# bibymaths/phoskintime

Measured on AMD Instinct MI355X. Metric: ODE-solve replicas/sec (32-state distributive, 14 tp), higher is better.
Workload: dtype f64

## Files before the change

### phoskintime_amd/csrc/pk_dist_fast.hpp

```cpp
#pragma once
#include "pk_dist_rows.hpp"
#include "pk_env.hpp"

namespace pk {

template <int G, int RPL>
__device__ __forceinline__ double site_sum(const double (&s)[RPL], int lane) { return gsum<G>(tree_sum(s), lane); }

enum { PK_DM_NONE = 0, PK_DM_SUM = 1, PK_DM_FULL = 2 };
__host__ __device__ __forceinline__ int dist_metric_class(const SolveArgs& A) {
  return !A.metric ? PK_DM_NONE : (A.metric_id == PK_METRIC_TOTAL_SIGNAL || A.metric_id == PK_METRIC_MEAN_ACTIVITY) ? PK_DM_SUM : PK_DM_FULL;
}
template <bool CLIP, bool NORM, bool FLAT, bool SOL, int MC>
struct DistFixed {
  static constexpr int SLOT_MC = MC;
  static constexpr bool LITERAL = false;
  __host__ __device__ static __forceinline__ bool clip(const SolveArgs&) { return CLIP; }
  __host__ __device__ static __forceinline__ bool normalize(const SolveArgs&) { return NORM; }
  __host__ __device__ static __forceinline__ bool flat(const SolveArgs&) { return FLAT; }
  __host__ __device__ static __forceinline__ bool sol(const SolveArgs&) { return SOL; }
  __host__ __device__ static __forceinline__ int mclass(const SolveArgs&) { return MC; }
  static bool matches(const SolveArgs& A) {
    return (A.clip != 0) == CLIP && (A.normalize != 0) == NORM && (A.flat != nullptr) == FLAT && (A.sol != nullptr) == SOL && dist_metric_class(A) == MC;
  }
};
struct DistAny {
  static constexpr int SLOT_MC = PK_DM_FULL;
  static constexpr bool LITERAL = true;
  __host__ __device__ static __forceinline__ bool clip(const SolveArgs& A) { return A.clip != 0; }
  __host__ __device__ static __forceinline__ bool normalize(const SolveArgs& A) { return A.normalize != 0; }
  __host__ __device__ static __forceinline__ bool flat(const SolveArgs& A) { return A.flat != nullptr; }
  __host__ __device__ static __forceinline__ bool sol(const SolveArgs& A) { return A.sol != nullptr; }
  __host__ __device__ static __forceinline__ int mclass(const SolveArgs& A) { return dist_metric_class(A); }
  static bool matches(const SolveArgs&) { return true; }
};
using DistSolSum = DistFixed<true, false, false, true, PK_DM_SUM>;
using DistSolOnly = DistFixed<true, false, false, true, PK_DM_NONE>;
using DistFlatOnly = DistFixed<true, false, true, false, PK_DM_NONE>;

template <int RPL, int MC, bool RES = false> constexpr int dist_fast_slots() {
  return MC == PK_DM_FULL ? 3 * RPL + (RES ? 4 : 6) : MC == PK_DM_SUM ? 2 * RPL + 1 : 2 * RPL;
}

template <int RPL, bool PARK, int NT> struct Parked;
template <int RPL, int NT> struct Parked<RPL, false, NT> {
  double v[3 * RPL + 6];
  __device__ __forceinline__ explicit Parked(double*) {}
  template <int K> __device__ __forceinline__ double get() const { return v[K]; }
  template <int K> __device__ __forceinline__ void set(double x) { v[K] = x; }
  __device__ __forceinline__ void fence() {}
};
template <int RPL, int NT> struct Parked<RPL, true, NT> {
  typedef __attribute__((address_space(3))) double lds_double;
  lds_double* base;
  __device__ __forceinline__ explicit Parked(double* lds) : base((lds_double*)lds + threadIdx.x) {}
  template <int K> __device__ __forceinline__ double get() const { return base[K * NT]; }
  template <int K> __device__ __forceinline__ void set(double x) { base[K * NT] = x; }
  __device__ __forceinline__ void fence() { asm volatile("" : "+v"(base)); }
};
template <int RPL, bool PARK, int NT = 256, class CFG = DistAny, bool RES = false>
constexpr size_t dist_fast_lds_bytes() { return PARK ? (size_t)(dist_fast_slots<RPL, CFG::SLOT_MC, RES>() + RPL) * NT * sizeof(double) : 0; }

constexpr int PK_DSCHED_K2 = 5, PK_DSCHED_K1 = 9;
constexpr int PK_HWREG_HW_ID = 4 | (31 << 11), PK_HWREG_HW_ID_WAVE = 4 | (3 << 11), PK_HWREG_XCC_ID = 20 | (31 << 11);

template <bool PACE> struct DistPace {
  __device__ __forceinline__ void enter(const SolveArgs&) {}
  __device__ __forceinline__ void step(int) const {}
};
template <> struct DistPace<true> {
  bool paced = false;
  __device__ __forceinline__ void enter(const SolveArgs& A) {
    const int sched = A.sched;
    if (sched != PK_DSCHED_OFF) {
      bool leader = false;
      if ((int)gridDim.x > A.R1) {
        if (sched & PK_DSCHED_LEAD_SLOT) leader = (int)blockIdx.x < A.R1 && __builtin_amdgcn_s_getreg(PK_HWREG_HW_ID_WAVE) == 0;
        if (sched & PK_DSCHED_LEAD_BLOCK) leader = leader || (int)blockIdx.x < A.R1 / 3;
      }
      if (leader) __builtin_amdgcn_s_setprio(3);
      paced = !leader && (sched & PK_DSCHED_LEVEL) != 0;
    }
  }
  __device__ __forceinline__ void step(const int k) const {
    if (paced) {
      if (__builtin_amdgcn_ballot_w64(k < PK_DSCHED_K2) != 0) __builtin_amdgcn_s_setprio(2);
      else if (__builtin_amdgcn_ballot_w64(k < PK_DSCHED_K1) != 0) __builtin_amdgcn_s_setprio(1);
      else __builtin_amdgcn_s_setprio(0);
    }
  }
};

struct DistTraceRec {
  unsigned long long t_entry, t_exit;
  unsigned block, hw_id, xcc_id, iters;
};
struct DistTraceBuf { DistTraceRec* rec; long long capacity; };
template <int TRACE> struct DistTrace;

template <int TRACE> struct DistWaveTrace {
  int witer = 0;
  __device__ __forceinline__ void enter() {
    const unsigned long long t0 = __builtin_amdgcn_s_memrealtime();
    const DistTraceBuf tb = DistTrace<TRACE>::get();
    if (threadIdx.x == 0 && tb.rec && (long long)blockIdx.x < tb.capacity) {
      DistTraceRec* r = tb.rec + blockIdx.x;
      r->t_entry = t0; r->t_exit = 0; r->block = blockIdx.x; r->iters = 0;
      r->hw_id = __builtin_amdgcn_s_getreg(PK_HWREG_HW_ID); r->xcc_id = __builtin_amdgcn_s_getreg(PK_HWREG_XCC_ID);
    }
  }
  __device__ __forceinline__ void step() { ++witer; }
  __device__ __forceinline__ void exit() const {
    int it = witer;
    for (int o = 32; o > 0; o >>= 1) { const int v = __shfl_xor(it, o); it = v > it ? v : it; }
    const DistTraceBuf tb = DistTrace<TRACE>::get();
    if (threadIdx.x == 0 && tb.rec && (long long)blockIdx.x < tb.capacity) {
      DistTraceRec* r = tb.rec + blockIdx.x;
      r->iters = (unsigned)it; r->t_exit = __builtin_amdgcn_s_memrealtime();
    }
  }
};
template <> struct DistWaveTrace<0> {
  __device__ __forceinline__ void enter() {}
  __device__ __forceinline__ void step() {}
  __device__ __forceinline__ void exit() const {}
};

template <int G, int RPL, int METHOD, bool PARK = false, int MINB = (PARK ? 2 : 1), int NT = 256, class CFG = DistAny, bool RES = false, int TRACE = 0>
__global__ __launch_bounds__(NT, MINB) void dist_fast_kernel(const SolveArgs A) {
  using Tab = ResolventTab<METHOD>;
  using Vec = Stg<RPL, RES>;
  static_assert(!TRACE || NT == 64, "the trace holds one record per workgroup: one wave each");
  DistWaveTrace<TRACE> trace;
  trace.enter();
  DistPace<PARK && NT == 64 && METHOD == PK_METHOD_LRP12> pace;
  pace.enter(A);
  extern __shared__ __align__(16) double park_lds[];
  Parked<RPL, PARK, NT> pk(park_lds);
  static_assert(dist_fast_lds_bytes<RPL, PARK, 64, CFG, RES>() * 4 * MINB <= 160 * 1024, "parked slots exceed the CU's LDS at this occupancy");
  constexpr int MCS = CFG::SLOT_MC;
  constexpr int NSL = dist_fast_slots<RPL, MCS, RES>(), FB = 3 * RPL + (RES ? 0 : 2);
  constexpr int K_SR = 0, K_DG = RPL, K_PS = 2 * RPL, K_PR = 3 * RPL, K_PP = 3 * RPL + 1, K_M1 = (MCS == PK_DM_FULL ? FB : 2 * RPL),
                K_M2 = FB + 1, K_MD = FB + 2, K_SH = FB + 3, K_Y = NSL;
  constexpr int RPB = NT / G;
  const int lane = lane_id();
  const int l = threadIdx.x & (G - 1);
  const long long rep = (long long)blockIdx.x * RPB + (threadIdx.x / G);
  if (rep >= A.B) return;
  const int n = A.n_sites, S = A.S, T = A.T;
  const int mclass = CFG::mclass(A);
  const double* __restrict__ th = A.theta + rep * A.P;

  const double cA = th[0], cB = th[1], cC = th[2];
  const bool isR = RES && l == 0, isP = RES && l == 1;
  const double w0 = isR ? cC : 1.0, k3 = isR ? cA : 0.0;
  double lsum = 0.0;
  static_for<RPL>([&](auto jc) {
    constexpr int j = decltype(jc)::value;
    const int i = l + G * j - (RES ? 2 : 0);
    const bool ok = i >= 0 && i < n;
    const double sr = ok ? th[4 + i] : 0.0;
    double dg = ok ? 1.0 + th[4 + n + i] : 1.0;
    if constexpr (RES && j == 0) dg = isR ? cB : isP ? -cC : dg;
    pk.template set<K_SR + j>(sr);
    pk.template set<K_DG + j>(dg);
    lsum += sr;
  });
  const double Dsum = th[3] + gsum<G>(lsum, lane);
  auto sites_only = [&](const auto& s) {
    double v[RPL];
#pragma unroll
    for (int j = 0; j < RPL; ++j) v[j] = s[j];
    v[0] = (isR || isP) ? 0.0 : v[0];
    return gsum<G>(tree_sum(v), lane);
  };

  const double* y0p = A.y0 + (A.y0_batched ? rep * S : 0);
  Vec y;
  if constexpr (!RES) { y.R() = y0p[0]; y.P() = y0p[1]; }
#pragma unroll
  for (int j = 0; j < RPL; ++j) {
    const int i = l + G * j;
    if constexpr (RES) y.s[j] = (i < S) ? y0p[i] : 0.0;
    else y.s[j] = (i < n) ? y0p[2 + i] : 0.0;
  }
  if constexpr (PARK) static_for<RPL>([&](auto jc) { constexpr int j = decltype(jc)::value; pk.template set<K_Y + j>(y.s[j]); });

  static_for<NSL - 2 * RPL>([&](auto kc) { pk.template set<K_PS + decltype(kc)::value>(0.0); });
  const int T5 = T > 5 ? T - 5 : 0;
  double* srow = CFG::sol(A) ? A.sol + rep * T * S + (RES ? 0 : 2) + l : nullptr;
  auto emit = [&](const int k, const Vec& v, auto nf) {
    constexpr bool nan_fill = decltype(nf)::value;
    double* fl = CFG::flat(A) ? A.flat + rep * A.F : nullptr;
    bool clip_now = CFG::clip(A);
    if constexpr (!CFG::LITERAL && !nan_fill) if (clip_now) clip_now = __builtin_amdgcn_ballot_w64(sign_or(v) < 0) != 0;
    auto val = [&](double x, int state) {
      if (nan_fill) return __builtin_nan("");
      double r = (CFG::LITERAL && CFG::clip(A)) ? ((x < 0.0) ? 0.0 : x) : x;
      if (CFG::normalize(A)) r *= 1.0 / y0p[state];
      return r;
    };
    Vec c = v;
    if constexpr (!CFG::LITERAL && !nan_fill) if (clip_now) {
      asm volatile("" : "+v"(c.s[Vec::tree_row(0)]));
      clip_rows(c);
    }
    double vR = 0.0, vP = 0.0;
    if constexpr (!RES) {
      vR = val(c.R(), 0); vP = val(c.P(), 1);
      if (l == 0) {
        if (CFG::sol(A)) { srow[-2] = vR; srow[-1] = vP; }
        if (CFG::flat(A)) { if (k >= 5) fl[k - 5] = vR; fl[T5 + k] = vP; }
      }
    }
    const bool masked = CFG::LITERAL || CFG::normalize(A);
    double vs[RPL];
    double loc = (!RES && l == 0) ? vR + vP : 0.0;
#pragma unroll
    for (int j = 0; j < RPL; ++j) {
      const int i = l + G * j;
      if constexpr (RES) {
        vs[j] = (i < S || !masked) ? val(c.s[j], i) : 0.0;
        if (i < S) {
          if (CFG::sol(A)) srow[G * j] = vs[j];
          if (CFG::flat(A)) if (j > 0 || i > 0 || k >= 5) fl[T5 + (i - 1) * T + k] = vs[j];
        }
      } else {
        vs[j] = (i < n || !masked) ? val(c.s[j], 2 + i) : 0.0;
        if (i < n) {
          if (CFG::sol(A)) srow[G * j] = vs[j];
          if (CFG::flat(A)) fl[T5 + T + i * T + k] = vs[j];
        }
      }
      loc += vs[j];
    }
    if (CFG::sol(A)) srow += S;
    if (mclass != PK_DM_NONE) {
      pk.template set<K_M1>(pk.template get<K_M1>() + loc);
      if constexpr (MCS == PK_DM_FULL) if (mclass == PK_DM_FULL) {
        double m2 = pk.template get<K_M2>(), mdyn = pk.template get<K_MD>(), shift = pk.template get<K_SH>();
        double prevR = 0.0, prevP = 0.0;
        if constexpr (!RES) { prevR = pk.template get<K_PR>(); prevP = pk.template get<K_PP>(); }
        if (k == 0) {
          shift = gsum<G>(loc, lane) / (2 + n);
          pk.template set<K_SH>(shift);
          prevR = vR; prevP = vP;
          static_for<RPL>([&](auto jc) { constexpr int j = decltype(jc)::value; pk.template set<K_PS + j>(vs[j]); });
        }
        static_for<RPL>([&](auto jc) {
          constexpr int j = decltype(jc)::value;
          const int i = l + G * j;
          const double xs = (i < (RES ? S : n)) ? vs[j] - shift : 0.0;
          m2 = __builtin_fma(xs, xs, m2);
          const double d = vs[j] - pk.template get<K_PS + j>();
          mdyn = __builtin_fma(d, d, mdyn);
          pk.template set<K_PS + j>(vs[j]);
        });
        if constexpr (!RES) {
          if (l == 0) {
            const double a = vR - shift, b = vP - shift;
            m2 = __builtin_fma(a, a, m2); m2 = __builtin_fma(b, b, m2);
            const double dR = vR - prevR, dP = vP - prevP;
            mdyn = __builtin_fma(dR, dR, mdyn); mdyn = __builtin_fma(dP, dP, mdyn);
          }
          pk.template set<K_PR>(vR); pk.template set<K_PP>(vP);
        }
        pk.template set<K_M2>(m2); pk.template set<K_MD>(mdyn);
      }
    }
  };
  auto finish = [&](const int status, const int acc, const int rej) {
    if (mclass != PK_DM_NONE) {
      const double L = 2.0 * T + (double)T * n;
      const double tot = gsum<G>(pk.template get<K_M1>(), lane);
      double m = tot;
      if (A.metric_id == PK_METRIC_MEAN_ACTIVITY) m = tot / L;
      if constexpr (MCS == PK_DM_FULL) if (mclass == PK_DM_FULL) {
        const double m2 = pk.template get<K_M2>(), mdyn = pk.template get<K_MD>(), shift = pk.template get<K_SH>();
        switch (A.metric_id) {
          case PK_METRIC_VARIANCE: { const double q = gsum<G>(m2, lane); const double ms = tot / L - shift; m = q / L - ms * ms; } break;
          case PK_METRIC_DYNAMICS: m = gsum<G>(mdyn, lane); break;
          default: { const double q = gsum<G>(m2, lane); m = sqrt(fmax(q + 2.0 * shift * tot - L * shift * shift, 0.0)); } break;
        }
      }
      if (l == 0) A.metric[rep] = m;
    }
    if (l == 0) {
      if (A.status) A.status[rep] = status;
      if (A.n_steps) { A.n_steps[2 * rep] = acc; A.n_steps[2 * rep + 1] = rej; }
    }
  };

  emit(0, y, std::false_type{});
  int status = PK_ST_OK, nacc = 0;
  if (T < 2) { trace.exit(); finish(status, 0, 0); return; }

  const double rtol = A.rtol, atol = A.atol;
  const DistNorm<G, RPL, RES> norm{rtol, atol, lane};
  auto rhs_of = [&](const Vec& Y, const double sg) {
    Vec f;
    if constexpr (RES) {
      const double Rb = bcast<G, 0>(Y.s[0]), Pb = bcast<G, 1>(Y.s[0]);
      static_for<RPL>([&](auto jc) {
        constexpr int j = decltype(jc)::value;
        const double sr = pk.template get<K_SR + j>(), dg = pk.template get<K_DG + j>();
        if constexpr (j == 0) f.s[0] = __builtin_fma(isP ? -Dsum : sr, Pb, __builtin_fma(-dg, isP ? Rb : Y.s[0], isP ? sg : k3));
        else f.s[j] = __builtin_fma(sr, Pb, -dg * Y.s[j]);
      });
    } else {
      f.R() = __builtin_fma(-cB, Y.R(), cA);
      f.P() = __builtin_fma(cC, Y.R(), __builtin_fma(-Dsum, Y.P(), sg));
      static_for<RPL>([&](auto jc) {
        constexpr int j = decltype(jc)::value;
        f.s[j] = __builtin_fma(pk.template get<K_SR + j>(), Y.P(), -pk.template get<K_DG + j>() * Y.s[j]);
      });
    }
    return f;
  };

  double tc = A.t[0];
  int k = 1;
  double te = A.t[1];
  double h;
  {
    double sg0;
    if constexpr (RES) sg0 = sites_only(y.s);
    else {
      double v[RPL];
#pragma unroll
      for (int j = 0; j < RPL; ++j) v[j] = y.s[j];
      sg0 = site_sum<G>(v, lane);
    }
    const Vec f0 = rhs_of(y, sg0);
    const double d0 = norm.group_max(y, y, y), d1 = norm.group_max(f0, y, y);
    h = step_h0(d0, d1, A.h0);
  }

  double winv[RPL], cw[RPL], omw[RPL], winvR, omwR, Cl, sinv, Scw, qq, qs, ws0;
  auto factor = [&](const double q) {
    qq = q;
    constexpr int X = RES ? 0 : 1;
    constexpr int NP = RPL + X, M0 = NP <= 5 ? NP : (NP + 1) / 2, M1 = NP - M0;
    double piv[NP];
    if constexpr (!RES) piv[0] = __builtin_fma(q, cB, 1.0);
    static_for<RPL>([&](auto jc) {
      constexpr int j = decltype(jc)::value;
      piv[X + j] = __builtin_fma(q, pk.template get<K_DG + j>(), 1.0);
    });
    if constexpr (RES) piv[0] = isP ? q : piv[0];
    {
      double a[M0], inv[M0];
#pragma unroll
      for (int i = 0; i < M0; ++i) a[i] = piv[i];
      chain_rcp<M0>(a, inv);
      if constexpr (!RES) winvR = inv[0];
#pragma unroll
      for (int i = X; i < M0; ++i) winv[i - X] = inv[i];
    }
    if constexpr (M1 > 0) {
      double a[M1], inv[M1];
#pragma unroll
      for (int i = 0; i < M1; ++i) a[i] = piv[M0 + i];
      chain_rcp<M1>(a, inv);
#pragma unroll
      for (int i = 0; i < M1; ++i) winv[M0 - X + i] = inv[i];
    }
    static_for<RPL>([&](auto jc) {
      constexpr int j = decltype(jc)::value;
      if constexpr (Tab::DIFFERENCE) {
        const double qw = q * winv[j];
        cw[j] = qw * pk.template get<K_SR + j>();
        omw[j] = qw * pk.template get<K_DG + j>();
      } else cw[j] = q * pk.template get<K_SR + j>() * winv[j];
    });
    if constexpr (!Tab::DIFFERENCE) Scw = gsum<G>(tree_sum(cw), lane);
    else if constexpr (!RES) {
      omwR = q * winvR * cB;
      Cl = tree_sum(cw);
      Scw = gsum<G>(Cl, lane);
    } else if constexpr (RPL > 1) {
      double rest[RPL - 1];
#pragma unroll
      for (int j = 1; j < RPL; ++j) rest[j - 1] = cw[j];
      Cl = tree_sum(rest);
      Scw = gsum<G>(Cl + cw[0], lane);
    } else {
      Cl = 0.0;
      Scw = gsum<G>(cw[0], lane);
    }
    sinv = fast_rcp(__builtin_fma(q, Dsum - Scw, 1.0));
    if constexpr (RES) {
      qs = q * sinv;
      ws0 = winv[0] * w0;
      winv[0] = isP ? 0.0 : winv[0];
      cw[0] = isP ? 1.0 : cw[0];
      if constexpr (Tab::DIFFERENCE) omw[0] = isP ? 1.0 : omw[0];
    }
  };
  double lam = 0.0;
  auto solve = [&](const Vec& r) {
    Vec u;
    double xR = 0.0;
    if constexpr (!RES) xR = r.R() * winvR;
    double t[RPL];
#pragma unroll
    for (int j = 0; j < RPL; ++j) t[j] = r.s[j] * winv[j];
    if constexpr (RES) {
      double in, tsum = 0.0;
      if constexpr (RPL > 1) {
        double rest[RPL - 1];
#pragma unroll
        for (int j = 1; j < RPL; ++j) rest[j - 1] = t[j];
        tsum = tree_sum(rest);
        in = __builtin_fma(r.s[0], ws0, tsum);
      } else in = r.s[0] * ws0;
      const double xP = gsum<G>(in, lane) * qs;
      if constexpr (Tab::DIFFERENCE && RPL > 1) lam = __builtin_fma(xP, Cl, tsum);
#pragma unroll
      for (int j = 0; j < RPL; ++j) u.s[j] = __builtin_fma(cw[j], xP, t[j]);
    } else {
      const double tsum = tree_sum(t);
      const double St = gsum<G>(tsum, lane);
      const double xP = __builtin_fma(qq, __builtin_fma(cC, xR, St), r.P()) * sinv;
      if constexpr (Tab::DIFFERENCE) lam = __builtin_fma(xP, Cl, tsum);
#pragma unroll
      for (int j = 0; j < RPL; ++j) u.s[j] = __builtin_fma(cw[j], xP, t[j]);
      u.R() = xR; u.P() = xP;
    }
    return u;
  };
  auto diff = [&](Vec& v) {
    double p[RPL];
#pragma unroll
    for (int j = 0; j < RPL; ++j) p[j] = omw[j] * v.s[j];
    if constexpr (RES) {
      double in, psum = 0.0;
      if constexpr (RPL > 1) {
        double rest[RPL - 1];
#pragma unroll
        for (int j = 1; j < RPL; ++j) rest[j - 1] = p[j];
        psum = tree_sum(rest);
        in = __builtin_fma(v.s[0], ws0, lam - psum);
      } else in = v.s[0] * ws0;
      const double xP = gsum<G>(in, lane) * qs;
#pragma unroll
      for (int j = 0; j < RPL; ++j) v.s[j] = __builtin_fma(-cw[j], xP, p[j]);
      if constexpr (RPL > 1) lam = __builtin_fma(-xP, Cl, psum);
    } else {
      const double psum = tree_sum(p);
      const double xR = v.R() * winvR;
      const double St = gsum<G>(lam - psum, lane);
      const double xP = __builtin_fma(qq, __builtin_fma(cC, xR, St), v.P()) * sinv;
#pragma unroll
      for (int j = 0; j < RPL; ++j) v.s[j] = __builtin_fma(-cw[j], xP, p[j]);
      lam = __builtin_fma(-xP, Cl, psum);
      v.R() *= omwR; v.P() -= xP;
    }
  };

  bool after_reject = false;
  auto state_bad = [&]() {
    double rows[RPL];
#pragma unroll
    for (int j = 0; j < RPL; ++j) rows[j] = y.s[j];
    if constexpr (PARK) {
      pk.fence();
      static_for<RPL>([&](auto jc) { constexpr int j = decltype(jc)::value; rows[j] = pk.template get<K_Y + j>(); });
    }
    bool b;
    if constexpr (RES) b = ((isR || isP) && nonfinite(rows[0])) || nonfinite(sites_only(rows));
    else b = (nonfinite(y.R())) || (nonfinite(y.P())) || (nonfinite(site_sum<G>(rows, lane)));
    return gmax<G>(b ? 1.0 : 0.0, lane);
  };
  auto coef_bad = [&]() {
    if constexpr (RES) {
      long long r2 = rep;
      asm volatile("" : "+v"(r2));
      const double* t2 = A.theta + r2 * A.P;
      return (nonfinite(t2[0])) || (nonfinite(t2[1])) || (nonfinite(t2[2]));
    } else return (nonfinite(cA)) || (nonfinite(cB)) || (nonfinite(cC));
  };
  int nsec = 0;
  __builtin_amdgcn_s_waitcnt(0x0F70);
  while (true) {
    bool nonfin = false;
    while (true) {
      trace.step();
      pace.step(k);
      const double tnx = A.t[k + 1 < T ? k + 1 : T - 1];
      const bool over = (CFG::LITERAL ? nacc + nsec : nsec) >= A.max_steps;
      const bool last = (tc + 1.0001 * h >= te);
      const double hs = last ? te - tc : ((tc + 2.0 * h > te) ? 0.5 * (te - tc) : h);
      if (over || !(hs > 1e-14 * max_abs_k(tc, 1e-3))) { status |= over ? PK_ST_MAXSTEPS : PK_ST_HMIN; break; }
      if constexpr (PARK) {
        pk.fence();
        static_for<RPL>([&](auto jc) { constexpr int j = decltype(jc)::value; y.s[j] = pk.template get<K_Y + j>(); });
      }
      factor(Tab::GAM * hs);

      Vec z;
      {
        Vec r = y;
        if constexpr (RES) r.s[0] = __builtin_fma(qq, k3, y.s[0]); else r.R() = __builtin_fma(qq, cA, y.R());
        z = solve(r);
        trk_axpy(z, -1.0, y);
      }
      Vec yn = y; trk_axpy(yn, Tab::B[0] / Tab::GAM, z);
      double err;
      if constexpr (Tab::DIFFERENCE) {
        z = solve(z);
        trk_axpy(yn, Tab::BN[0] / Tab::GAM, z);
        static_for<Tab::NS - 2>([&](auto mc) {
          constexpr int m = 1 + decltype(mc)::value;
          diff(z);
          trk_axpy(yn, Tab::BN[m] / Tab::GAM, z);
        });
        constexpr double e1 = (Tab::E[1] < 0.0 ? -Tab::E[1] : Tab::E[1]) / Tab::GAM;
        if constexpr (CFG::LITERAL) err = e1 * norm.group_max(z, y, yn); else err = e1 * norm.err_norm(z, y, yn);
      } else {
        Vec u6;
        static_for<Tab::NS - 1>([&](auto kc) {
          constexpr int kk = 1 + decltype(kc)::value;
          constexpr double bk = Tab::B[kk] / Tab::GAM, ek = Tab::E[kk] / Tab::GAM;
          z = solve(z);
          trk_axpy(yn, bk, z);
          if constexpr (kk == 1) u6 = trk_scale(ek, z); else trk_axpy(u6, ek, z);
        });
        if constexpr (CFG::LITERAL) err = norm.group_max(u6, y, yn); else err = norm.err_norm(u6, y, yn);
      }
      const bool acc = (err <= 1.0);
      if constexpr (PARK) {
        if (acc) {
          static_for<RPL>([&](auto jc) { constexpr int j = decltype(jc)::value; pk.template set<K_Y + j>(yn.s[j]); });
          if constexpr (!CFG::LITERAL) tc += hs;
        }
#pragma unroll
        for (int j = 0; j < RPL; ++j) y.s[j] = yn.s[j];
        #pragma unroll
        for (int x = 0; x < Vec::X; ++x) y.s[RPL + x] = acc ? yn.s[RPL + x] : y.s[RPL + x];
      } else {
        if (acc) {
          y = yn;
          if constexpr (!CFG::LITERAL) tc += hs;
        }
      }
      if constexpr (CFG::LITERAL) {
        if (err != err || err > 1e300) {
          ++nsec; after_reject = true; h = 0.1 * hs;
          if (state_bad() != 0.0 || coef_bad() || (nonfinite(Dsum)) || (nonfinite(Scw))) {
            status |= PK_ST_NONFINITE; break;
          }
          continue;
        }
      } else {
        ++nsec;
        if (__builtin_expect(err != err || err > 1e300, 0)) { after_reject = true; h = 0.1 * hs; nonfin = true; break; }
      }
      const float e32 = (float)min_raw_k(max_raw_k(err, 1e-30), 1e30);
      const double finv = step_growth((double)__builtin_amdgcn_exp2f(__builtin_amdgcn_logf(e32) * (float)(-1.0 / Tab::Q)));
      double hnew = hs * finv;
      const bool land = acc && last;
      if constexpr (CFG::LITERAL) { nacc += acc ? 1 : 0; nsec += acc ? 0 : 1; }
      else nacc += (int)acc;
      if (acc && after_reject) hnew = min_raw(hnew, hs);
      after_reject = !acc;
      if constexpr (CFG::LITERAL) tc = land ? te : (acc ? tc + hs : tc);
      h = (land && hs < h) ? max_raw(hnew, h) : hnew;
      if (land) {
        if constexpr (!CFG::LITERAL) tc = te;
        te = tnx;
        asm volatile("" : "+v"(te));
        emit(k, y, std::false_type{});
        ++k;
      }
      if (k >= T) break;
    }
    if (CFG::LITERAL || !nonfin) break;
    if (state_bad() != 0.0 || coef_bad() || (nonfinite(Dsum)) || (nonfinite(Scw))) {
      status |= PK_ST_NONFINITE; break;
    }
  }
  const int nrej = CFG::LITERAL ? nsec : nsec - nacc;
  if (status != PK_ST_OK)
    for (; k < T; ++k) emit(k, y, std::true_type{});
  trace.exit();
  finish(status, nacc, nrej);
}

}
```

Before: 254.9 million.

## Rescale site rows so resolvent solve and difference steps need fewer multiplies

For parked, difference-method variants at certain rows-per-lane counts, the site states are rescaled by their source rates (clamped away from denormals) so the per-stage solve and diff reduce to a single dot product plus one FMA per row. The dot product is split into two independent chains. The scaled increments are mapped back to the original variables before the error norm, which reloads y from LDS. This aims to shorten the dependent FMA chain in the inner Newton-free stages, at the cost of extra factor work, more registers (g, ic, is) and possible rounding differences from the scaling.

Measured after the change: 261.4 million (median of 6 runs). 1.03x the previous value.

```diff
diff --git a/phoskintime_amd/csrc/pk_dist_fast.hpp b/phoskintime_amd/csrc/pk_dist_fast.hpp
--- a/phoskintime_amd/csrc/pk_dist_fast.hpp
+++ b/phoskintime_amd/csrc/pk_dist_fast.hpp
@@ -126,10 +126,18 @@
   __device__ __forceinline__ void exit() const {}
 };
 
+template <int METHOD, int RPL, bool PARK, bool RES> constexpr bool dist_scaled() {
+  return PARK && ResolventTab<METHOD>::DIFFERENCE && (RES ? (RPL == 6 || RPL == 8) : (RPL >= 5 && RPL <= 7));
+}
+constexpr double PK_DIST_SCALE_MIN = 0x1p-600;
+
 template <int G, int RPL, int METHOD, bool PARK = false, int MINB = (PARK ? 2 : 1), int NT = 256, class CFG = DistAny, bool RES = false, int TRACE = 0>
 __global__ __launch_bounds__(NT, MINB) void dist_fast_kernel(const SolveArgs A) {
   using Tab = ResolventTab<METHOD>;
   using Vec = Stg<RPL, RES>;
+  constexpr bool SCL = dist_scaled<METHOD, RPL, PARK, RES>();
+  constexpr int J0 = RES ? 1 : 0;
+  static_assert(!SCL || RPL - J0 >= 2, "the scaled rows' dot product runs on two chains");
   static_assert(!TRACE || NT == 64, "the trace holds one record per workgroup: one wave each");
   DistWaveTrace<TRACE> trace;
   trace.enter();
@@ -335,8 +343,18 @@
     const double d0 = norm.group_max(y, y, y), d1 = norm.group_max(f0, y, y);
     h = step_h0(d0, d1, A.h0);
   }
-
-  double winv[RPL], cw[RPL], omw[RPL], winvR, omwR, Cl, sinv, Scw, qq, qs, ws0;
+  double is[RPL];
+  if constexpr (SCL) static_for<RPL>([&](auto jc) {
+    constexpr int j = decltype(jc)::value;
+    if constexpr (j >= J0) {
+      const double sr = pk.template get<K_SR + j>();
+      const double s = !(fabs(sr) < PK_DIST_SCALE_MIN) ? sr : (sr == 0.0 && y.s[j] == 0.0) ? 0.0 : PK_DIST_SCALE_MIN;
+      pk.template set<K_SR + j>(s);
+      is[j] = s != 0.0 ? 1.0 / s : 0.0;
+    }
+  });
+
+  double winv[RPL], cw[RPL], omw[RPL], g[RPL], ic[RPL], winvR, omwR, Cl, sinv, Scw, qq, qs, ws0;
   auto factor = [&](const double q) {
     qq = q;
     constexpr int X = RES ? 0 : 1;
@@ -367,14 +385,24 @@
     }
     static_for<RPL>([&](auto jc) {
       constexpr int j = decltype(jc)::value;
-      if constexpr (Tab::DIFFERENCE) {
+      if constexpr (SCL) {
+        cw[j] = winv[j] * pk.template get<K_SR + j>();
+        omw[j] = (q * winv[j]) * pk.template get<K_DG + j>();
+        if constexpr (j >= J0) {
+          g[j] = winv[j] * cw[j];
+          ic[j] = piv[X + j] * is[j];
+        }
+      } else if constexpr (Tab::DIFFERENCE) {
         const double qw = q * winv[j];
         cw[j] = qw * pk.template get<K_SR + j>();
         omw[j] = qw * pk.template get<K_DG + j>();
       } else cw[j] = q * pk.template get<K_SR + j>() * winv[j];
     });
     if constexpr (!Tab::DIFFERENCE) Scw = gsum<G>(tree_sum(cw), lane);
-    else if constexpr (!RES) {
+    else if constexpr (SCL) {
+      if constexpr (!RES) omwR = q * winvR * cB;
+      Scw = q * gsum<G>(tree_sum(cw), lane);
+    } else if constexpr (!RES) {
       omwR = q * winvR * cB;
       Cl = tree_sum(cw);
       Scw = gsum<G>(Cl, lane);
@@ -391,16 +419,49 @@
     sinv = fast_rcp(__builtin_fma(q, Dsum - Scw, 1.0));
     if constexpr (RES) {
       qs = q * sinv;
+      if constexpr (SCL) qs *= q;
       ws0 = winv[0] * w0;
+      if constexpr (SCL) cw[0] = isP ? winv[0] : cw[0]; else cw[0] = isP ? 1.0 : cw[0];
       winv[0] = isP ? 0.0 : winv[0];
-      cw[0] = isP ? 1.0 : cw[0];
       if constexpr (Tab::DIFFERENCE) omw[0] = isP ? 1.0 : omw[0];
     }
   };
   double lam = 0.0;
-  auto solve = [&](const Vec& r) {
+  auto gdot = [&](const Vec& v) {
+    if constexpr (SCL) {
+      constexpr int H = (RPL + J0) / 2;
+      double a, b = g[H] * v.s[H];
+      if constexpr (RES) a = v.s[0] * ws0; else a = g[0] * v.s[0];
+#pragma unroll
+      for (int j = 1; j < H; ++j) a = __builtin_fma(g[j], v.s[j], a);
+#pragma unroll
+      for (int j = H + 1; j < RPL; ++j) b = __builtin_fma(g[j], v.s[j], b);
+      return a + b;
+    } else return 0.0;
+  };
+  auto xq_of = [&](const Vec& v, double& xR, double& xP) {
+    if constexpr (RES) return gsum<G>(gdot(v), lane) * qs;
+    else {
+      xR = v.R() * winvR;
+      xP = __builtin_fma(qq, __builtin_fma(cC, xR, gsum<G>(gdot(v), lane)), v.P()) * sinv;
+      return qq * xP;
+    }
+  };
+  auto solve = [&](const Vec& r, auto first) {
     Vec u;
     double xR = 0.0;
+    if constexpr (SCL) {
+      double xP = 0.0;
+      const double xq = xq_of(r, xR, xP);
+      if constexpr (RES) u.s[0] = __builtin_fma(cw[0], xq, r.s[0] * winv[0]);
+      else { u.R() = xR; u.P() = xP; }
+#pragma unroll
+      for (int j = J0; j < RPL; ++j) {
+        if constexpr (decltype(first)::value) u.s[j] = __builtin_fma(-omw[j], r.s[j], xq);
+        else u.s[j] = __builtin_fma(-omw[j], r.s[j], r.s[j] + xq);
+      }
+      return u;
+    }
     if constexpr (!RES) xR = r.R() * winvR;
     double t[RPL];
 #pragma unroll
@@ -430,6 +491,15 @@
     return u;
   };
   auto diff = [&](Vec& v) {
+    if constexpr (SCL) {
+      double xR = 0.0, xP = 0.0;
+      const double xq = xq_of(v, xR, xP);
+      if constexpr (RES) v.s[0] = __builtin_fma(-cw[0], xq, omw[0] * v.s[0]);
+      else { v.R() *= omwR; v.P() -= xP; }
+#pragma unroll
+      for (int j = J0; j < RPL; ++j) v.s[j] = __builtin_fma(omw[j], v.s[j], -xq);
+      return;
+    }
     double p[RPL];
 #pragma unroll
     for (int j = 0; j < RPL; ++j) p[j] = omw[j] * v.s[j];
@@ -502,19 +572,41 @@
       {
         Vec r = y;
         if constexpr (RES) r.s[0] = __builtin_fma(qq, k3, y.s[0]); else r.R() = __builtin_fma(qq, cA, y.R());
-        z = solve(r);
-        trk_axpy(z, -1.0, y);
-      }
-      Vec yn = y; trk_axpy(yn, Tab::B[0] / Tab::GAM, z);
+        if constexpr (SCL) {
+#pragma unroll
+          for (int j = J0; j < RPL; ++j) r.s[j] = y.s[j] * ic[j];
+          z = solve(r, std::true_type{});
+#pragma unroll
+          for (int j = 0; j < Vec::NR; ++j) if (j < J0 || j >= RPL) z.s[j] -= y.s[j];
+        } else {
+          z = solve(r, std::false_type{});
+          trk_axpy(z, -1.0, y);
+        }
+      }
+      Vec yn = y;
+      if constexpr (SCL) {
+#pragma unroll
+        for (int j = J0; j < RPL; ++j) yn.s[j] = 0.0;
+      }
+      trk_axpy(yn, Tab::B[0] / Tab::GAM, z);
       double err;
       if constexpr (Tab::DIFFERENCE) {
-        z = solve(z);
+        z = solve(z, std::false_type{});
         trk_axpy(yn, Tab::BN[0] / Tab::GAM, z);
         static_for<Tab::NS - 2>([&](auto mc) {
           constexpr int m = 1 + decltype(mc)::value;
           diff(z);
           trk_axpy(yn, Tab::BN[m] / Tab::GAM, z);
         });
+        if constexpr (SCL) {
+          pk.fence();
+          static_for<RPL - J0>([&](auto jc) { constexpr int j = J0 + decltype(jc)::value; y.s[j] = pk.template get<K_Y + j>(); });
+#pragma unroll
+          for (int j = J0; j < RPL; ++j) {
+            yn.s[j] = __builtin_fma(cw[j], yn.s[j], y.s[j]);
+            z.s[j] *= cw[j];
+          }
+        }
         constexpr double e1 = (Tab::E[1] < 0.0 ? -Tab::E[1] : Tab::E[1]) / Tab::GAM;
         if constexpr (CFG::LITERAL) err = e1 * norm.group_max(z, y, yn); else err = e1 * norm.err_norm(z, y, yn);
       } else {
@@ -522,7 +614,7 @@
         static_for<Tab::NS - 1>([&](auto kc) {
           constexpr int kk = 1 + decltype(kc)::value;
           constexpr double bk = Tab::B[kk] / Tab::GAM, ek = Tab::E[kk] / Tab::GAM;
-          z = solve(z);
+          z = solve(z, std::false_type{});
           trk_axpy(yn, bk, z);
           if constexpr (kk == 1) u6 = trk_scale(ek, z); else trk_axpy(u6, ek, z);
         });
```
